# LarsDoorenbos/ccdm-stochastic-segmentation

Hardware: AMD Instinct MI355X
Metric: segmentation samples/sec, LIDC 128x128 T=250 (higher is better)
Workload: dtype f32 (conv products as split fp16 hi/lo x3 on MFMA, fp32 accumulate)

## Files before the change

### ccdm_stochastic_segmentation_amd/csrc/ccdm_conv.hip

```cpp
#include "ccdm_common.h"
#include "ccdm_conv_common.h"

#include <cmath>
#include <cstdlib>
#include <type_traits>
#include <vector>

namespace ccdm {


constexpr int min_waves(int mi, int ni, int prec, int ckt, int threads) {
    if (threads > 512) return 3;
    if (prec != CCDM_PREC_F32 && ckt >= 32) return 2;
    return mi * ni <= 2 ? 3 : (mi * ni <= 4 ? 2 : 1);
}

template <int PREC, int CKT, int KS, int STRIDE, int TH, int TW, int WAVES, int MI, int NI, int KSP = 1, bool UP2 = false, bool SKWT = false>
__global__ __launch_bounds__(WAVES * KSP * 64, min_waves(MI, NI, PREC, CKT, WAVES * KSP * 64)) void k_conv(const ConvK k) {
    constexpr int NT = WAVES * KSP * 64;
    static_assert(KSP == 1 || KSP == KS, "tap split is by kernel row");
    static_assert(!UP2 || (KS == 3 && STRIDE == 1 && KSP == 1 && (NI == 1 || NI == 4) && PREC != CCDM_PREC_F32), "sub-pixel form: 3x3, stride 1, F16X3, one phase or all four");
    constexpr int NTAP = UP2 ? 4 : KS * KS;
    constexpr int CK = CKT, PIXB = conv_pixb(PREC, CKT);
    constexpr int KST = CK / 16;
// ... 5 lines not shown
    constexpr int PXW = NT / QPP;
    static_assert(PXW % CW == 0, "a pass must cover whole core rows");
    constexpr int RPP = PXW / CW;
    constexpr int NCORE = (HHt + RPP - 1) / RPP;
    constexpr int ECOLS = HWt - CW > 0 ? HWt - CW : 1;
    constexpr int EDGE_ITEMS = HHt * (HWt - CW) * QPP;
    constexpr int NEDGE = (EDGE_ITEMS + NT - 1) / NT;
    constexpr bool ROW_UNIFORM = (CW * QPP) % 64 == 0;
    constexpr int NITEM = NCORE + NEDGE;
    static_assert(NITEM <= 32, "validity mask is 32 bits");
    constexpr bool SKW = SKWT && PREC != CCDM_PREC_F32 && KS == 3 && STRIDE == 1 && TW == 32 && NI == 1 && KSP == 1 && !UP2 && CKT == 16;
    constexpr int CKS = 32, PIXS = conv_pixb(CCDM_PREC_F16X3, CKS), QPS = CKS / 4;
    constexpr int NITEM_S = SKW ? TH * TW * QPS / NT : 0;
    constexpr int NITEM_R = NITEM_S > NITEM ? NITEM_S : NITEM;
    static_assert(!SKW || (TH * TW * QPS) % NT == 0, "a wide skip chunk tiles the block");
    constexpr int A_BYTES = (HP * PIXB + 15) / 16 * 16;
    constexpr int G = NI * FRAG_ITEMS;
    constexpr int NB4 = PREC == CCDM_PREC_F32 ? 0 : NTAP * KST * G;
    constexpr int NITEM_B = (NB4 + NT - 1) / NT;
    constexpr bool B_MULTI = NT % G == 0;
    static_assert(PREC == CCDM_PREC_F32 || B_MULTI || G % NT == 0, "B slabs must tile the block");
    constexpr int MB = B_MULTI ? NT / G : 1, DB = B_MULTI ? 1 : G / NT;

    const ccdm_conv_args& a = k.a;
    extern __shared__ __attribute__((aligned(16))) char smem[];
    const int C = a.C0 + a.C1;
    float2* ab = reinterpret_cast<float2*>(smem);
    char* halo_b = smem + (a.stats0 ? (size_t)C * 8 : 0);
    float* halo = reinterpret_cast<float*>(halo_b);
    f32x4* ldsB = reinterpret_cast<f32x4*>(halo_b + A_BYTES);
// ... 188 lines not shown
        const unsigned dst0 = (unsigned)(size_t)(skwc ? halo_b + TH * TW * PIXS : reinterpret_cast<char*>(ldsB));
        unsigned lane_ = lane;
        asm volatile("" : "+v"(lane_));
#pragma unroll
        for (int i = 0; i < MAXU; ++i) {
            const unsigned u = (unsigned)wave_all + (unsigned)(i * NWV);
            if (u < nunit) {
                const unsigned ts = u / UPS, part = u % UPS;
                const unsigned slab = skwc ? ts * wks : (ts / KST) * wtap + (ts % KST) * wks;
                const char* src = wq + (((size_t)slab + part * (FRAG_ITEMS / 2)) << 4) + (lane_ << 4);
                __builtin_amdgcn_global_load_lds(reinterpret_cast<const __attribute__((address_space(1))) void*>(reinterpret_cast<unsigned long long>(src)),
                                                 reinterpret_cast<__attribute__((address_space(3))) void*>(dst0 + u * (unsigned)(FRAG_BYTES / 2)), 16, 0, 0);
            }
        }
    };
    auto commit_body = [&](auto GN_, auto ACT_, int c0) {
        constexpr bool GN = decltype(GN_)::value, ACT = decltype(ACT_)::value;
        unsigned t_ = tid;
        asm volatile("" : "+v"(t_));
        const int tq = t_ % QPP, px = (t_ / QPP) % CW;
        float2 t0 = make_float2(1.f, 0.f), t1 = t0, t2 = t0, t3 = t0;
        if (GN) { const int c = c0 + 4 * tq; t0 = ab[c]; t1 = ab[c + 1]; t2 = ab[c + 2]; t3 = ab[c + 3]; }
        constexpr bool F16 = PREC != CCDM_PREC_F32;
        constexpr float PS = F16 ? ACT_PRESCALE : 1.0f;
        if (GN && !ACT && F16) { t0.x *= PS; t0.y *= PS; t1.x *= PS; t1.y *= PS; t2.x *= PS; t2.y *= PS; t3.x *= PS; t3.y *= PS; }
        auto act = [&](const float x) {
            if (!ACT) return (GN || !F16) ? x : x * PS;
            return x * __builtin_amdgcn_rcpf(1.0f / PS + __builtin_amdgcn_exp2f(fmaf(x, -1.4426950408889634f, F16 ? -4.0f : 0.0f)));
        };
        static_assert(ACT_PRESCALE == 16.0f, "the exp2 bias above is log2(ACT_PRESCALE)");
        auto put = [&](auto MASKED_, const f32x4 r, const bool ok, const int hp) {
            constexpr bool MASKED = decltype(MASKED_)::value;
// ... 46 lines not shown
        } else {
#pragma unroll
            for (int i = 0; i < NCORE; ++i)
                if ((i + 1) * RPP <= HHt || rip + i * RPP < HHt)
                    put(std::true_type{}, reg[i], xok[0] & (((rowmask[0] >> i) & 1u) != 0u), hp0 + i * RPP * HWt);
        }
#pragma unroll
        for (int j = 0; j < NEDGE; ++j) {
            const unsigned e = t_ + j * NT;
            if (e < (unsigned)EDGE_ITEMS) {
                const unsigned side = (e / QPP) % ECOLS, row = e / (ECOLS * QPP);
                const int hx = side < (unsigned)PAD ? (int)side : CW + (int)side;
                put(std::true_type{}, reg[NCORE + j], ((evalid[0] >> j) & 1u) != 0u, (int)row * HWt + hx);
            }
        }
        if (PREC != CCDM_PREC_F32 && !BDMA) {
#pragma unroll
            for (int i = 0; i < NITEM_B; ++i) {
                const int j = (int)t_ + i * NT;
                if ((i + 1) * NT <= NB4 || j < NB4) ldsB[j] = regB[i];
            }
        }
    };
    auto commit_skipw = [&]() {
        if constexpr (SKW) {
            unsigned t_ = tid;
            asm volatile("" : "+v"(t_));
            const int tq = t_ % QPS, px = t_ / QPS;
            typedef unsigned u32x2 __attribute__((ext_vector_type(2)));
#pragma unroll
            for (int i = 0; i < NITEM_S; ++i) {
// ... 2 lines not shown
                const float lim = ok ? __builtin_inff() : 0.f;
                const float v0 = __builtin_amdgcn_fmed3f(r[0] * ACT_PRESCALE, -lim, lim), v1 = __builtin_amdgcn_fmed3f(r[1] * ACT_PRESCALE, -lim, lim);
                const float v2 = __builtin_amdgcn_fmed3f(r[2] * ACT_PRESCALE, -lim, lim), v3 = __builtin_amdgcn_fmed3f(r[3] * ACT_PRESCALE, -lim, lim);
                u32x2 hi, lo;
                unsigned h0, l0, h1, l1;
                split2_f16(v0, v1, h0, l0);
                split2_f16(v2, v3, h1, l1);
                hi[0] = h0; hi[1] = h1; lo[0] = l0; lo[1] = l1;
                char* dd = halo_b + (i * TW + px) * PIXS + 8 * tq;
                *reinterpret_cast<u32x2*>(dd) = hi;
                *reinterpret_cast<u32x2*>(dd + 2 * CKS) = lo;
            }
            if (!BDMA) reinterpret_cast<f32x4*>(halo_b + TH * TW * PIXS)[t_] = regB[0];
        }
    };
    auto commit = [&](const int ch) {
        const bool sk = ch >= nchunk_main;
        if (SKW && skw && sk) { commit_skipw(); return; }
        const int c0 = (sk ? ch - nchunk_main : ch) * CK;
        const bool gn = has_gn && !sk, act = a.act == CCDM_ACT_SILU && !sk;
        if (gn && act) commit_body(std::true_type{}, std::true_type{}, c0);
        else if (gn) commit_body(std::true_type{}, std::false_type{}, c0);
        else if (act) commit_body(std::false_type{}, std::true_type{}, c0);
        else commit_body(std::false_type{}, std::false_type{}, c0);
    };

    f32x16 acc[MI][NI];
    const int adv_y = k.slices / k.tiles_x, adv_x = k.slices % k.tiles_x;
    auto advance = [&](int& ch, int& ty, int& tx) {
        if (++ch == nchunk) {
            ch = 0; tx += adv_x; ty += adv_y;
            if (tx >= k.tiles_x) { tx -= k.tiles_x; ++ty; }
        }
    };
    int chunk = 0, cur_ty = slice / k.tiles_x, cur_tx = slice % k.tiles_x;
    int pf_ch = 0, pf_ty = cur_ty, pf_tx = cur_tx;
    issue(pf_ch, pf_ty, pf_tx);
    advance(pf_ch, pf_ty, pf_tx);
    __builtin_amdgcn_sched_barrier(0);
#pragma unroll
    for (int ni = 0; ni < NI; ++ni) {
        const bool cv = tile_of(ni) * 32 + (lane & 31) < a.Cout;
        float add = a.bias ? raw_bias[ni] : 0.f;
        if (a.emb_off >= 0) add += raw_emb[ni];
        epi_add[ni] = (cv && krow == 0) ? add : 0.f;
        if (!cv) epi_wsc[ni] = 1.0f;
    }
    if (has_gn) gn_affine_block(a, n, emb_row, gpf, reinterpret_cast<f64x2*>(halo_b), ab, blockDim.x);
    auto iterate = [&]() {
        if (chunk == 0) {
#pragma unroll
            for (int mi = 0; mi < MI; ++mi)
#pragma unroll
                for (int ni = 0; ni < NI; ++ni)
#pragma unroll
                    for (int r = 0; r < 16; ++r) acc[mi][ni][r] = 0.0f;
        }
        issueB(chunk);
        __syncthreads();
        if constexpr (BDMA) {
#pragma unroll
            for (int i = 0; i < NITEM_R; ++i) asm volatile("" : "+v"(reg[i]));
            issueB_dma(chunk);
        }
        commit(chunk);
        __syncthreads();
        issue(pf_ch, pf_ty, pf_tx);
        advance(pf_ch, pf_ty, pf_tx);

        const bool skc = chunk >= nchunk_main;
        const int c0 = (skc ? chunk - nchunk_main : chunk) * CK;
        if (PREC == CCDM_PREC_F32) {
            const float* wc = reinterpret_cast<const float*>(skc ? a.skip_w : a.w) + ((size_t)(c0 >> 1) * k.ntiles + nt0) * 64 + lane;
            const size_t wtap = (size_t)(k.cin_pad >> 1) * k.ntiles * 64;
#pragma unroll
            for (int tap = 0; tap < KS * KS; ++tap) {
                if (skc && tap != (KS * KS) / 2) continue;
                const int toff = ((tap / KS) * HWt + (tap % KS)) * PIX_F32;
                const float* wt = wc + (skc ? 0 : tap * wtap);
#pragma unroll 4
                for (int kk = 0; kk < CK / 2; ++kk) {
                    float av[MI];
#pragma unroll
                    for (int mi = 0; mi < MI; ++mi) av[mi] = halo[base[mi] + toff + 2 * kk];
// ... 100 lines not shown
                            for (int mi = 0; mi < MI; ++mi) {
                                acc[mi][ni] = __builtin_amdgcn_mfma_f32_32x32x16_f16(al[0][mi], wh, acc[mi][ni], 0, 0, 0);
                                acc[mi][ni] = __builtin_amdgcn_mfma_f32_32x32x16_f16(ah[0][mi], wl, acc[mi][ni], 0, 0, 0);
                                acc[mi][ni] = __builtin_amdgcn_mfma_f32_32x32x16_f16(ah[0][mi], wh, acc[mi][ni], 0, 0, 0);
                            }
                        }
                    }
            } else if (UP2) {
                walk(std::integral_constant<int, 4>{}, [&](int t) { return ((t >> 1) * HWt + (t & 1)) * PIXB; }, [&](int t) { return t; });
            } else if (KSP > 1) {
                walk(std::integral_constant<int, KS>{}, [&](int u) { return (krow * HWt + u) * PIXB; }, [&](int u) { return krow * KS + u; });
            } else {
                walk(std::integral_constant<int, KS * KS>{}, [&](int tap) { return ((tap / KS) * HWt + (tap % KS)) * PIXB; }, [&](int tap) { return tap; });
            }
        }

        if (chunk == nchunk - 1) {
            const int oy0 = cur_ty * TH, ox0 = cur_tx * TW;
            int lane_ = lane;
            asm volatile("" : "+v"(lane_));
            if (fast_epi) {
                __syncthreads();
                const int cq = lane_ & 7, prow = lane_ >> 3;
#pragma unroll
                for (int ni = 0; ni < NI; ++ni) {
                    if (KSP > 1 && ni > 0) __syncthreads();
                    const int co4 = tile_of(ni) * 32 + 4 * cq;
                    const int dy = phase_of(ni) >> 1, dx = phase_of(ni) & 1;
                    const bool cv4 = co4 < a.Cout;
                    const int eH = UP2 ? Hc : aHout, eW = UP2 ? Wc : aWout;
                    const bool full = oy0 + TH <= eH && ox0 + TW <= eW && tile_of(ni) * 32 + 32 <= aCout;
                    constexpr int RS_FIRST = MI * 4 > 4 ? 4 : MI * 4;
                    f32x4 rs[MI * 4];
                    unsigned lane_off = ((unsigned)(UP2 ? 2 * prow : prow) * (unsigned)aCout + (unsigned)co4) << 2;
                    asm volatile("" : "+v"(lane_off));
                    auto row_of = [&](const int j) { return oy0 + wave * (MI * 32 / TW) + (j * 8) / TW; };
                    auto row_base = [&](const int j) {
                        if (UP2) return (unsigned)(((2 * row_of(j) + dy) * aWout + 2 * (ox0 + (j * 8) % TW) + dx) * aCout) << 2;
                        return (unsigned)((row_of(j) * aWout + ox0 + (j * 8) % TW) * aCout) << 2;
                    };
                    auto pix_of = [&](const int oy, const int ox) {
                        return UP2 ? (unsigned)((2 * oy + dy) * aWout + 2 * ox + dx) : (unsigned)(oy * aWout + ox);
                    };
                    double t1[4] = {0.0, 0.0, 0.0, 0.0}, t2[4] = {0.0, 0.0, 0.0, 0.0};
                    auto epi_ni = [&](auto FULL_, auto RESID_) {
                    constexpr bool FULL = decltype(FULL_)::value, RESID = decltype(RESID_)::value;
                    auto load_resid = [&](const int j0, const int j1) {
#pragma unroll
                        for (int j = j0; j < j1; ++j) {
                            if (KSP > 1 && j % KSP != krow) continue;
                            if (FULL) rs[j] = load16_uniform_base(reinterpret_cast<const char*>(residn) + row_base(j), lane_off);
                            else {
                                const int oy = min(row_of(j), eH - 1), ox = min(ox0 + (j * 8) % TW + prow, eW - 1);
                                const int cc = min(co4, aCout - 4);
                                rs[j] = *reinterpret_cast<const f32x4*>(reinterpret_cast<const char*>(residn) +
                                                                        ((pix_of(oy, ox) * (unsigned)aCout + (unsigned)cc) << 2));
                            }
                        }
                    };
                    if (RESID) load_resid(0, RS_FIRST);
                    constexpr bool EXACT3 = KS == 1 && RESID && PREC != CCDM_PREC_F32;
                    float addq[4] = {0.f, 0.f, 0.f, 0.f};
                    if (EXACT3) {
#pragma unroll
                        for (int e = 0; e < 4; ++e) addq[e] = __shfl(epi_add[ni], 4 * cq + e);
                    }
                    {
                        const float add = EXACT3 ? 0.f : epi_add[ni], wsc = epi_wsc[ni];
#pragma unroll
                        for (int mi = 0; mi < MI; ++mi)
#pragma unroll
                            for (int r = 0; r < 16; ++r) {
                                const int pl = mi * 32 + (r & 3) + 8 * (r >> 2) + 4 * (lane_ >> 5);
                                epi[pl * EPS + (lane_ & 31)] = PREC == CCDM_PREC_F32 ? acc[mi][ni][r] + add : fmaf(acc[mi][ni][r], wsc, add);
                            }
                    }
                    if (KSP > 1) __syncthreads();
                    const float* epi0 = reinterpret_cast<const float*>(halo_b) + wave * (MI * 32 * EPS);
                    {
#pragma unroll
                        for (int j = 0; j < MI * 4; ++j) {
                            if (j == RS_FIRST && RESID) load_resid(RS_FIRST, MI * 4);
                            if (KSP > 1 && j % KSP != krow) continue;
                            const int pl = j * 8 + prow;
                            f32x4 v = *reinterpret_cast<const f32x4*>(epi0 + pl * EPS + 4 * cq);
#pragma unroll
                            for (int g = 1; g < KSP; ++g)
                                v += *reinterpret_cast<const f32x4*>(epi0 + g * (WAVES * MI * 32 * EPS) + pl * EPS + 4 * cq);
                            if (EXACT3) {
#pragma unroll
                                for (int e = 0; e < 4; ++e) v[e] = (float)((double)v[e] + ((double)addq[e] + (double)rs[j][e]));
                            } else if (RESID) v += rs[j];
                            if (FULL) {
                                store16_uniform_base(reinterpret_cast<char*>(outn) + row_base(j), lane_off, v);
#pragma unroll
                                for (int e = 0; e < 4; ++e) { const double d = v[e]; t1[e] += d; t2[e] = fma(d, d, t2[e]); }
                            } else {
                                const int oy = row_of(j), ox = ox0 + (j * 8) % TW + prow;
                                if (cv4 && oy < eH && ox < eW) {
                                    *reinterpret_cast<f32x4*>(reinterpret_cast<char*>(outn) +
                                                              ((pix_of(oy, ox) * (unsigned)aCout + (unsigned)co4) << 2)) = v;
#pragma unroll
                                    for (int e = 0; e < 4; ++e) { const double d = v[e]; t1[e] += d; t2[e] = fma(d, d, t2[e]); }
                                }
                            }
                        }
                    }
                    };
                    if (a.resid) { if (full) epi_ni(std::true_type{}, std::true_type{}); else epi_ni(std::false_type{}, std::true_type{}); }
                    else { if (full) epi_ni(std::true_type{}, std::false_type{}); else epi_ni(std::false_type{}, std::false_type{}); }
                    {
                        const bool b2 = (lane_ >> 5) & 1, b1 = (lane_ >> 4) & 1, b0 = (lane_ >> 3) & 1;
                        double u[4], w[2];
#pragma unroll
                        for (int i = 0; i < 4; ++i) u[i] = (b2 ? t2[i] : t1[i]) + __shfl_xor(b2 ? t1[i] : t2[i], 32);
#pragma unroll
                        for (int i = 0; i < 2; ++i) w[i] = (b1 ? u[2 + i] : u[i]) + __shfl_xor(b1 ? u[i] : u[2 + i], 16);
                        st[ni] += (b0 ? w[1] : w[0]) + __shfl_xor(b0 ? w[0] : w[1], 8);
                    }
                }
            } else {
#pragma unroll
            for (int ni = 0; ni < NI; ++ni) {
                const int co = (nt0 + ni) * 32 + (lane_ & 31);
                const bool cv = co < a.Cout;
                const float add = epi_add[ni], wsc = epi_wsc[ni];
                double t1 = 0.0, t2 = 0.0;
#pragma unroll
                for (int mi = 0; mi < MI; ++mi) {
                    const int pb = (wave * MI + mi) * 32 + 4 * (lane_ >> 5);
#pragma unroll
                    for (int r = 0; r < 16; ++r) {
                        const int p = pb + (r & 3) + 8 * (r >> 2);
                        const int oy = oy0 + p / TW, ox = ox0 + p % TW;
                        if (cv && oy < a.Hout && ox < a.Wout) {
                            const size_t idx = ((size_t)(n * a.Hout + oy) * a.Wout + ox) * a.Cout + co;
                            float v;
                            if (KS == 1 && PREC != CCDM_PREC_F32 && a.resid) v = (float)((double)(acc[mi][ni][r] * wsc) + ((double)add + (double)a.resid[idx]));
                            else {
                                v = (PREC == CCDM_PREC_F32 ? acc[mi][ni][r] : acc[mi][ni][r] * wsc) + add;
                                if (a.resid) v += a.resid[idx];
                            }
                            a.out[idx] = v;
                            const double d = v;
                            t1 += d;
                            t2 = fma(d, d, t2);
                        }
                    }
                }
                const bool h = lane_ >> 5;
                st[ni] += (h ? t2 : t1) + __shfl_xor(h ? t1 : t2, 32);
            }
            }
        }
        advance(chunk, cur_ty, cur_tx);
    };
    for (int it = 0; it < n_iter; ++it) iterate();

    if (a.out_stats) {
        __syncthreads();
        double* red = reinterpret_cast<double*>(halo_b);
        const int ch = fast_epi ? 4 * (lane & 7) + ((lane >> 3) & 3) : lane & 31, comp = lane >> 5;
#pragma unroll
        for (int ni = 0; ni < NI; ++ni) red[((wave_all * NI + ni) * 32 + ch) * 2 + comp] = st[ni];
        __syncthreads();
        constexpr int NFOLD = UP2 && NI == 4 ? 4 : 1;
        for (int i = tid; i < NI / NFOLD * 32; i += NT) {
            const int ni = (i >> 5) * NFOLD, l = i & 31;
            double t1 = 0.0, t2 = 0.0;
            for (int f = 0; f < NFOLD; ++f) gn_fold_waves(red, ni + f, NI, WAVES * KSP, l, t1, t2);
            const int co = tile_of(ni) * 32 + l;
            if (co < a.Cout) {
// ... 183 lines not shown
        return 0;
    }
    if (conv1x1_eligible(a, p.slices)) {
        conv1x1_plan(a, p);
        return 0;
    }
    if (conv_takes_ks(a)) {
        CCDM_REQUIRE(conv_ks_describe(a, p), "conv_ks: geometry not built");
        return 0;
    }
    p.kernel = CCDM_CONV_KERNEL_GENERAL;
    const int HP = ((g.TH - 1) * a.stride + a.ksize) * ((g.TW - 1) * a.stride + a.ksize);
    const int ck = chunk_ck(a, g);
    p.chunk = ck;
    p.skip_wide = (a.skip0 && prec == CCDM_PREC_F16X3 && a.ksize == 3 && a.stride == 1 && !a.up && g.TW == 32 && NI == 1 && ck == 16 &&
                   a.SC0 % 32 == 0 && a.SC1 % 32 == 0 && !(a.prec >> 8)) ? 1 : 0;
    {
        const int SC = a.SC0 + a.SC1;
        const bool chan_ok = a.C0 % ck == 0 && a.C1 % ck == 0 && (!a.skip0 || (a.SC0 % ck == 0 && a.SC1 % ck == 0 && SC > 0));
        p.core_unmasked = ((up2 ? a.Win : Wc) % (g.TW * a.stride) == 0 && chan_ok) ? 1 : 0;
    }
    CCDM_REQUIRE(a.C1 == 0 || a.C0 % ck == 0, "conv: first source has %d channels; a concatenated input must split at a multiple of the %d-channel chunk", a.C0, ck);
    CCDM_REQUIRE(a.SC1 == 0 || a.SC0 % ck == 0, "conv: first skip source has %d channels; a concatenated input must split at a multiple of the %d-channel chunk", a.SC0, ck);
    CCDM_REQUIRE((p.cin_pad + p.cin_pad_skip) / ck <= 64, "conv: %d input (+%d skip) channels make more than 64 chunks of %d (chunk descriptors live in the 64 lanes of a register)",
                 p.cin_pad, p.cin_pad_skip, ck);
    size_t lds = (size_t)HP * conv_pixb(prec, ck);
    lds = (lds + 15) / 16 * 16;
    if (prec != CCDM_PREC_F32) lds += (size_t)(up2 ? 4 : a.ksize * a.ksize) * (ck / 16) * NI * FRAG_BYTES;
    p.tap_split = tap_split(a, g) ? 1 : 0;
    const int ksp = p.tap_split ? 3 : 1;
    const size_t red = (size_t)g.waves * ksp * NI * 32 * 16;
// ... 36 lines not shown
        if (rck) return rck;
        CCDM_CHECK_LAUNCH("conv_ks");
        return 0;
    }
    ConvK k;
    k.a = a;
    k.cin_pad = p.cin_pad;
    k.cin_pad_skip = p.cin_pad_skip;
    k.ntiles = p.ntiles;
    k.slices = p.slices;
    k.tiles_x = cdiv(a.up == 2 ? a.Win : a.Wout, p.g.TW);
    k.tiles_y = cdiv(a.up == 2 ? a.Hin : a.Hout, p.g.TH);
    k.skip_wide = p.skip_wide;
    k.wscale = wscale;
    k.core_unmasked = p.core_unmasked;
    const int prec = a.prec & 255;
    const dim3 grid(p.grid_x, p.grid_y);
    const int rc = prec == CCDM_PREC_F32 ? launch_prec<CCDM_PREC_F32>(k, p.g, p.ntiles_per_block, p.chunk, grid, (size_t)p.lds_bytes, s)
                   : prec == CCDM_PREC_F16 ? launch_prec<CCDM_PREC_F16>(k, p.g, p.ntiles_per_block, p.chunk, grid, (size_t)p.lds_bytes, s)
                                           : launch_prec<CCDM_PREC_F16X3>(k, p.g, p.ntiles_per_block, p.chunk, grid, (size_t)p.lds_bytes, s);
    if (rc) return rc;
    CCDM_CHECK_LAUNCH("conv");
    return 0;
}

}

extern "C" int ccdm_conv_slices(int Hout, int Wout, int stride, int ksize) {
    (void)ksize;
    return ccdm::conv_slices(Hout, Wout, stride);
// ... 115 lines not shown
```

### ccdm_stochastic_segmentation_amd/csrc/ccdm_conv1x1.hip

```cpp
#include "ccdm_common.h"
#include "ccdm_conv_common.h"

#include <cstdlib>

namespace ccdm {

__device__ __forceinline__ float epi_bias_resid(float acc, float wsc, float add, float rs, bool resid) {
    if (!resid) return fmaf(acc, wsc, add);
    return (float)fma((double)acc, (double)wsc, (double)add + (double)rs);
}

struct Conv1x1K {
    const float* in;
    const void* w;
    const float* wscale;
    const float* bias;
    const float* resid;
    float* out;
    double* out_stats;
    int C, Cout, HW, slices, ntiles, px_per_block;
    ccdm_conv_args a;
};

template <int KSB, int MAXT, bool GN>
// ... 202 lines not shown
        if (t + 1 >= ntb || nt + 1 >= nt_real) break;
        issueB(0, nt + 2);
        tile(1, nt + 1);
    }
}

static int conv1x1_px_per_block(const ccdm_conv_args& a, int slices) {
    const int HW = a.Hout * a.Wout;
    if (a.out_stats) return (HW % (slices * 32) == 0 && HW / slices <= 512) ? HW / slices : 0;
    for (int p = 128; p >= 32; p >>= 1)
        if (HW % p == 0) return p;
    return 0;
}

bool conv1x1_eligible(const ccdm_conv_args& a, int slices) {
    if (a.prec != CCDM_PREC_F16X3) return false;
    if (a.ksize != 1 || a.stride != 1 || a.up || a.act != CCDM_ACT_NONE || a.film || a.skip0 || a.emb_off >= 0 || a.in1) return false;
    const int HW = a.Hout * a.Wout;
    if (a.C0 % 16 || a.Cout % 32 || a.C0 > CCDM_MAX_CHANNELS) return false;
    const int ppb = conv1x1_px_per_block(a, slices);
    if (a.stats0 && ppb > 128) return false;
    return ppb > 0 && HW <= 16384;
}

void conv1x1_plan(const ccdm_conv_args& a, ConvPlan& p) {
    const int HW = a.Hout * a.Wout, ppb = conv1x1_px_per_block(a, p.slices);
    p.slices = HW / ppb;
    p.tile_h = 1; p.tile_w = ppb;
    p.chunk = 16;
    p.block = ppb / 32 * 64;
    p.lds_bytes = a.stats0 ? a.C0 * 8 + (a.C0 > p.block ? a.C0 : p.block) * 16 : 0;
// ... 38 lines not shown
```

### ccdm_stochastic_segmentation_amd/csrc/ccdm_conv_common.h

```cpp
#pragma once
#include "ccdm_common.h"
#include "ccdm_gn.h"

namespace ccdm {

static constexpr float ACT_PRESCALE = 16.0f;

constexpr int PIX_F32 = 33;
constexpr int conv_pixb(int prec, int ck) { return prec == CCDM_PREC_F32 ? PIX_F32 * 4 : ck * 4 + 16; }
constexpr int EPI_ROW = 36;
constexpr int FRAG_ITEMS = 128, FRAG_BYTES = FRAG_ITEMS * 16;

typedef const __attribute__((address_space(1))) char* gptr_t;
__device__ __forceinline__ f32x4 load16_uniform_base(const char* base, unsigned voff) {
    const unsigned long long v = reinterpret_cast<unsigned long long>(base);
    const unsigned lo = __builtin_amdgcn_readfirstlane((unsigned)v), hi = __builtin_amdgcn_readfirstlane((unsigned)(v >> 32));
    gptr_t g = reinterpret_cast<gptr_t>(((unsigned long long)hi << 32) | lo);
    return *reinterpret_cast<const __attribute__((address_space(1))) f32x4*>(g + voff);
}

__device__ __forceinline__ f32x4 load16_global(const char* p) {
    return *reinterpret_cast<const __attribute__((address_space(1))) f32x4*>(reinterpret_cast<unsigned long long>(p));
}

// ... 8 lines not shown
__device__ __forceinline__ void split2_f16(const float a, const float b, unsigned& hi, unsigned& lo) {
    float la, lb;
    asm("v_cvt_pk_f16_f32 %0, %1, %2" : "=v"(hi) : "v"(a), "v"(b));
    asm("v_fma_mix_f32 %0, %1, -1.0, %2 op_sel:[0,0,0] op_sel_hi:[1,0,0]" : "=v"(la) : "v"(hi), "v"(a));
    asm("v_fma_mix_f32 %0, %1, -1.0, %2 op_sel:[1,0,0] op_sel_hi:[1,0,0]" : "=v"(lb) : "v"(hi), "v"(b));
    asm("v_cvt_pk_f16_f32 %0, %1, %2" : "=v"(lo) : "v"(la), "v"(lb));
}

struct ConvK {
    ccdm_conv_args a;
    int cin_pad, ntiles, slices, tiles_x, tiles_y;
    int cin_pad_skip;
    int skip_wide;
    const float* wscale;
    int core_unmasked;
};

struct ConvPlan : ccdm_conv_plan_info {
    ConvGeo g;
    int cin_pad, cin_pad_skip;
    size_t wscale_off;
};
int conv_plan(const ccdm_conv_args& a, ConvPlan& p);

bool conv1x1_eligible(const ccdm_conv_args& a, int slices);
void conv1x1_plan(const ccdm_conv_args& a, ConvPlan& p);
int launch_conv1x1(const ccdm_conv_args& a, const ConvPlan& p, const float* wscale, hipStream_t s);

bool conv_ks_eligible(const ccdm_conv_args& a);
int conv_ks_slices(const ccdm_conv_args& a);
// ... 8 lines not shown
```

### ccdm_stochastic_segmentation_amd/csrc/ccdm_conv_ks.hip

```cpp
#include "ccdm_common.h"
#include "ccdm_conv_common.h"

namespace ccdm {

struct ConvKS {
    ccdm_conv_args a;
    const float* wscale;
    int ntiles;
    int tiles_x, tiles_y;
    int C, SC;
    int nks_m, nks_s;
    int pitch_m, pitch_s;
    int lgq_m, lgq_s;
    int nit_m, nit_s;
    int skip_off;
    int nstep;
    int red_off;
};

constexpr int KS_NT = 512, KS_NW = 8, KS_PART_BYTES = 8 * 2 * 4 * 64 * 16;
constexpr int ks_bq(int ni) { return ni == 1 ? 10 : (ni == 2 ? 6 : (ni == 3 ? 4 : 2)); }

template <int STRIDE, bool GNACT, int NITM, int NITS, int NI = 1>
__global__ __launch_bounds__(KS_NT, NI == 1 ? 2 : 1) void k_conv_ks(const ConvKS k) {
// ... 344 lines not shown

static int pow2_lg_quads(int nks) {
    const int q = 4 * nks;
    return q <= 16 ? 4 : (q <= 32 ? 5 : 6);
}

static int conv_ks_ni(const ccdm_conv_args& a) {
    if (a.Hout * a.Wout <= 128) return 1;
    const int nt = a.Cout / 32;
    for (int ni = 4; ni > 1; --ni)
        if (nt % ni == 0) return ni;
    return 1;
}

static bool conv_ks_plan(const ccdm_conv_args& a, ConvKS& k, size_t& lds, int& NI) {
    if (a.prec != CCDM_PREC_F16X3) return false;
    if (a.ksize != 3 || a.up || a.film || (a.stride != 1 && a.stride != 2)) return false;
    if ((a.stats0 != nullptr) != (a.act == CCDM_ACT_SILU)) return false;
    if (a.Hout % 8 || a.Wout % 8 || a.Hout * a.Wout > 256) return false;
    if (a.Cout % 32) return false;
    const int C = a.C0 + a.C1, SC = a.skip0 ? a.SC0 + a.SC1 : 0;
    if (C > 256 || SC > 256 || (a.stride == 2 && a.skip0)) return false;
    NI = conv_ks_ni(a);
    if (NI > 1 && ((a.stride == 1) != (a.stats0 != nullptr))) return false;
    k.a = a;
    k.C = C; k.SC = SC;
    k.nks_m = cdiv(C, 16); k.nks_s = cdiv(SC, 16);
    k.pitch_m = conv_pixb(CCDM_PREC_F16X3, 16 * k.nks_m); k.pitch_s = conv_pixb(CCDM_PREC_F16X3, 16 * k.nks_s);
    k.lgq_m = pow2_lg_quads(k.nks_m); k.lgq_s = SC ? pow2_lg_quads(k.nks_s) : 6;
    const int HWt = 7 * a.stride + 3, HP = HWt * HWt;
    k.nit_m = cdiv(cdiv(HP, 64 >> k.lgq_m), KS_NW);
// ... 76 lines not shown
```

### ccdm_stochastic_segmentation_amd/csrc/ccdm_upconv.hip

```cpp
#include "ccdm_common.h"
#include "ccdm_conv_common.h"

#include <algorithm>

namespace ccdm {

struct UpK {
    const float* in;
    const void* w;
    const float* wscale;
    const float* bias;
    float* out;
    double* out_stats;
    int N, Hin, Win, Cout, ntiles, slices, tiles_x, tiles_y, ctb;
};

constexpr int UP_TH = 8, UP_HH = UP_TH + 2;
constexpr int UP_EPI_BYTES = 4 * 32 * EPI_ROW * 4;
constexpr int UP_CTB_MAX = 2;
constexpr int UP_BD = 2;

template <int C, int TW> struct UpGeo {
    static constexpr int PIXB = conv_pixb(CCDM_PREC_F16X3, C), QPP = C / 4, KS16 = C / 16, NF = KS16 * 4;
    static constexpr int HW = TW + 2, HP = UP_HH * HW, MT = UP_TH * TW / 32;
// ... 173 lines not shown
                o[1] = red[((w * UP_CTB_MAX + c) * 32 + l) * 2 + 1];
            }
        } else {
            for (int i = tid; i < k.ctb * 32; i += 256) {
                const int c = i >> 5, l = i & 31;
                double a1 = 0.0, a2 = 0.0;
                gn_fold_waves(red, c, UP_CTB_MAX, 4, l, a1, a2);
                double* o = k.out_stats + (((size_t)n * k.slices + slice) * Cout + (ct0 + c) * 32 + l) * 2;
                o[0] = a1; o[1] = a2;
            }
        }
    }
}

bool upconv_eligible(const ccdm_conv_args& a) {
    if (a.prec != CCDM_PREC_F16X3 || a.up != 2) return false;
    if (a.C1 || a.in1 || a.stats0 || a.act != CCDM_ACT_NONE || a.film || a.emb_off >= 0 || a.resid || a.skip0 || a.fine_slices) return false;
    if (!(a.C0 == 32 || a.C0 == 64 || a.C0 == 96 || a.C0 == 128) || a.Cout % 32) return false;
    return a.Hin % UP_TH == 0 && (a.Win % 16 == 0 || a.Win == 8);
}

void upconv_plan(const ccdm_conv_args& a, ConvPlan& p) {
    p.kernel = CCDM_CONV_KERNEL_UPCONV;
    p.tile_h = UP_TH; p.tile_w = a.Win == 8 ? 8 : 16;
    p.chunk = a.C0;
    const int ctiles = a.Cout / 32;
    p.ntiles_per_block = (ctiles % 2 == 0 && (long)a.N * p.slices * (ctiles / 2) >= 512) ? 2 : 1;
    p.grid_x = a.N * p.slices; p.grid_y = ctiles / p.ntiles_per_block; p.block = 256;
    const int a_bytes = UP_HH * (p.tile_w + 2) * conv_pixb(CCDM_PREC_F16X3, a.C0);
    p.lds_bytes = p.ntiles_per_block == 1 ? std::max(a_bytes, UP_EPI_BYTES) : a_bytes + UP_EPI_BYTES;
}
// ... 39 lines not shown
```

### ccdm_stochastic_segmentation_amd/hip.py

```python
from __future__ import annotations

import ctypes as C
import os
import subprocess
from typing import Optional

_HERE = os.path.dirname(os.path.abspath(__file__))
ROOT = os.path.dirname(_HERE)
LIB_PATH = os.environ.get("CCDM_LIB") or os.path.join(_HERE, "libccdm_hip.so")
CSRC = os.path.join(_HERE, "csrc")
SOURCES = ["ccdm_conv.hip", "ccdm_conv_ks.hip", "ccdm_upconv.hip", "ccdm_stem.hip", "ccdm_head.hip", "ccdm_conv1x1.hip", "ccdm_misc.hip", "ccdm_attention.hip", "ccdm_attn_block.hip", "ccdm_sampler.hip", "ccdm_known.hip", "ccdm_guided.hip", "ccdm_metrics.hip", "ccdm_range.hip", "ccdm_resample.hip", "ccdm_engine.hip", "ccdm_vote.hip", "ccdm_segeval.hip", "ccdm_segexport.hip", "ccdm_csscore.hip", "ccdm_segcalib.hip", "ccdm_segboundary.hip", "ccdm_contourf.hip", "ccdm_uncscore.hip", "ccdm_lidcscore.hip", "ccdm_surfdist.hip", "ccdm_lesions.hip", "ccdm_lesionmatch.hip", "ccdm_findings.hip", "ccdm_modes.hip", "ccdm_consensus.hip", "ccdm_bound.hip"]
HIPCC_FLAGS = ["--offload-arch=gfx950", "-O3", "-std=c++17", "-ffp-contract=off", "-mllvm", "-amdgpu-mfma-vgpr-form=1", "-fPIC", "-shared"]

ACT_NONE, ACT_SILU = 0, 1
RESAMPLE_AVGPOOL2, RESAMPLE_NEAREST_UP2 = 0, 1
ATTENTION_FORCE_VALU = 256
ATTENTION_VALU_WIDTHS = (4, 8, 12, 16, 24, 32, 48, 64)
DIAG_GENERAL_KERNEL = 2048 << 8
PREC_F32, PREC_F16X3 = 0, 1
PREC_F16 = 2
STEP_SAMPLE, STEP_LAST_CONFIDENCE, STEP_LAST_MAJORITY, STEP_LAST_KEEP, STEP_SOFTMAX_ONLY = 0, 1, 2, 3, 4
SLOT_IDLE = -1
SLOT_GUIDE_EVIDENCE, SLOT_GUIDE_KNOWN = 1, 2
BOUND_IDLE = -1
STATS_MAX_SLICES = 64
F16X3_LIMIT = 4094.0
STATS_FOLD_SLICES = 16
ABI_VERSION = 11
MAX_CLASSES = 255
CSSCORE_MAX_LABELS = 64
POST_DIAG_MANY = 256


# ... 435 lines not shown
```

### include/ccdm_hip.h

```cpp
#ifndef CCDM_HIP_H
#define CCDM_HIP_H

#include <stddef.h>
#include <stdint.h>

#ifdef __cplusplus
extern "C" {
#endif

#define CCDM_ABI_VERSION 11
#define CCDM_MAX_CHANNELS 1024
#define CCDM_STATS_MAX_SLICES 64
#define CCDM_STATS_FOLD_SLICES 16

int ccdm_version(void);
const char* ccdm_last_error_string(void);

int ccdm_gn_stats(const float* x , int N, int HW, int C, int slices,
                  double* stats , void* stream);

enum { CCDM_ACT_NONE = 0, CCDM_ACT_SILU = 1 };
enum { CCDM_PREC_F32 = 0,
       CCDM_PREC_F16X3 = 1,
       CCDM_PREC_F16 = 2 };

#define CCDM_DIAG_GENERAL_KERNEL (2048 << 8)

typedef struct ccdm_conv_args {
    const float* in0; const float* in1; int32_t C0; int32_t C1;
    const double* stats0; const double* stats1; int32_t slices0; int32_t slices1;
    const float* gamma; const float* beta;
    float eps; int32_t act;
    int32_t film; int32_t film_off;
    int32_t N, Hin, Win, Hout, Wout;
    int32_t ksize;
    int32_t stride;
    int32_t up;
    const void* w; const float* bias; int32_t Cout; int32_t prec;
    const float* emb_table; int32_t emb_stride; int32_t emb_off;
    const int32_t* emb_row_of_sample;
    const int32_t* step_ptr;
// ... 355 lines not shown
```

Before: 95.00.

## Process two output tiles per weight chunk to reuse staged weights in conv

For F16X3 3x3 stride-1 convs with TW=32, MI=2, NI=1, the tile loop now walks tile pairs. Each channel chunk's weight slab is staged into LDS once and used for both tiles, which keep separate accumulators. This removes the repeated weight writeback for the second tile, at the cost of doubling accumulator registers, which can reduce occupancy. A diagnostic flag restores the single-tile walk, and the other eligibility checks mask that flag out.

```diff
diff --git a/ccdm_stochastic_segmentation_amd/csrc/ccdm_conv.hip b/ccdm_stochastic_segmentation_amd/csrc/ccdm_conv.hip
--- a/ccdm_stochastic_segmentation_amd/csrc/ccdm_conv.hip
+++ b/ccdm_stochastic_segmentation_amd/csrc/ccdm_conv.hip
@@ -43,6 +43,7 @@
     constexpr int NITEM_S = SKW ? TH * TW * QPS / NT : 0;
     constexpr int NITEM_R = NITEM_S > NITEM ? NITEM_S : NITEM;
     static_assert(!SKW || (TH * TW * QPS) % NT == 0, "a wide skip chunk tiles the block");
+    constexpr bool PAIR = PREC == CCDM_PREC_F16X3 && CKT == 16 && KS == 3 && STRIDE == 1 && TW == 32 && MI == 2 && NI == 1 && KSP == 1 && !UP2 && !SKWT;
     constexpr int A_BYTES = (HP * PIXB + 15) / 16 * 16;
     constexpr int G = NI * FRAG_ITEMS;
     constexpr int NB4 = PREC == CCDM_PREC_F32 ? 0 : NTAP * KST * G;
@@ -261,8 +262,8 @@
             }
         }
     };
-    auto commit_body = [&](auto GN_, auto ACT_, int c0) {
-        constexpr bool GN = decltype(GN_)::value, ACT = decltype(ACT_)::value;
+    auto commit_body = [&](auto GN_, auto ACT_, auto WB_, int c0) {
+        constexpr bool GN = decltype(GN_)::value, ACT = decltype(ACT_)::value, WB = decltype(WB_)::value;
         unsigned t_ = tid;
         asm volatile("" : "+v"(t_));
         const int tq = t_ % QPP, px = (t_ / QPP) % CW;
@@ -339,7 +340,7 @@
                 put(std::true_type{}, reg[NCORE + j], ((evalid[0] >> j) & 1u) != 0u, (int)row * HWt + hx);
             }
         }
-        if (PREC != CCDM_PREC_F32 && !BDMA) {
+        if (PREC != CCDM_PREC_F32 && !BDMA && WB) {
 #pragma unroll
             for (int i = 0; i < NITEM_B; ++i) {
                 const int j = (int)t_ + i * NT;
@@ -372,18 +373,18 @@
             if (!BDMA) reinterpret_cast<f32x4*>(halo_b + TH * TW * PIXS)[t_] = regB[0];
         }
     };
-    auto commit = [&](const int ch) {
+    auto commit = [&](const int ch, auto WB_) {
         const bool sk = ch >= nchunk_main;
         if (SKW && skw && sk) { commit_skipw(); return; }
         const int c0 = (sk ? ch - nchunk_main : ch) * CK;
         const bool gn = has_gn && !sk, act = a.act == CCDM_ACT_SILU && !sk;
-        if (gn && act) commit_body(std::true_type{}, std::true_type{}, c0);
-        else if (gn) commit_body(std::true_type{}, std::false_type{}, c0);
-        else if (act) commit_body(std::false_type{}, std::true_type{}, c0);
-        else commit_body(std::false_type{}, std::false_type{}, c0);
+        if (gn && act) commit_body(std::true_type{}, std::true_type{}, WB_, c0);
+        else if (gn) commit_body(std::true_type{}, std::false_type{}, WB_, c0);
+        else if (act) commit_body(std::false_type{}, std::true_type{}, WB_, c0);
+        else commit_body(std::false_type{}, std::false_type{}, WB_, c0);
     };
 
-    f32x16 acc[MI][NI];
+    f32x16 accs[PAIR ? 2 : 1][MI][NI];
     const int adv_y = k.slices / k.tiles_x, adv_x = k.slices % k.tiles_x;
     auto advance = [&](int& ch, int& ty, int& tx) {
         if (++ch == nchunk) {
@@ -391,7 +392,7 @@
             if (tx >= k.tiles_x) { tx -= k.tiles_x; ++ty; }
         }
     };
-    int chunk = 0, cur_ty = slice / k.tiles_x, cur_tx = slice % k.tiles_x;
+    int cur_ch = 0, cur_ty = slice / k.tiles_x, cur_tx = slice % k.tiles_x;
     int pf_ch = 0, pf_ty = cur_ty, pf_tx = cur_tx;
     issue(pf_ch, pf_ty, pf_tx);
     advance(pf_ch, pf_ty, pf_tx);
@@ -405,27 +406,28 @@
         if (!cv) epi_wsc[ni] = 1.0f;
     }
     if (has_gn) gn_affine_block(a, n, emb_row, gpf, reinterpret_cast<f64x2*>(halo_b), ab, blockDim.x);
-    auto iterate = [&]() {
-        if (chunk == 0) {
-#pragma unroll
-            for (int mi = 0; mi < MI; ++mi)
-#pragma unroll
-                for (int ni = 0; ni < NI; ++ni)
-#pragma unroll
-                    for (int r = 0; r < 16; ++r) acc[mi][ni][r] = 0.0f;
-        }
-        issueB(chunk);
+    auto clear = [&](auto& acc) {
+#pragma unroll
+        for (int mi = 0; mi < MI; ++mi)
+#pragma unroll
+            for (int ni = 0; ni < NI; ++ni)
+#pragma unroll
+                for (int r = 0; r < 16; ++r) acc[mi][ni][r] = 0.0f;
+    };
+    auto stage = [&](auto SECOND_, const int chunk, auto&& prefetch) {
+        constexpr bool SECOND = decltype(SECOND_)::value;
+        if (!SECOND) issueB(chunk);
         __syncthreads();
         if constexpr (BDMA) {
 #pragma unroll
             for (int i = 0; i < NITEM_R; ++i) asm volatile("" : "+v"(reg[i]));
             issueB_dma(chunk);
         }
-        commit(chunk);
+        commit(chunk, std::integral_constant<bool, !SECOND>{});
         __syncthreads();
-        issue(pf_ch, pf_ty, pf_tx);
-        advance(pf_ch, pf_ty, pf_tx);
-
+        prefetch();
+    };
+    auto matrix = [&](auto& acc, const int chunk) {
         const bool skc = chunk >= nchunk_main;
         const int c0 = (skc ? chunk - nchunk_main : chunk) * CK;
         if (PREC == CCDM_PREC_F32) {
@@ -556,148 +558,184 @@
                 walk(std::integral_constant<int, KS * KS>{}, [&](int tap) { return ((tap / KS) * HWt + (tap % KS)) * PIXB; }, [&](int tap) { return tap; });
             }
         }
-
-        if (chunk == nchunk - 1) {
-            const int oy0 = cur_ty * TH, ox0 = cur_tx * TW;
-            int lane_ = lane;
-            asm volatile("" : "+v"(lane_));
-            if (fast_epi) {
-                __syncthreads();
-                const int cq = lane_ & 7, prow = lane_ >> 3;
-#pragma unroll
-                for (int ni = 0; ni < NI; ++ni) {
-                    if (KSP > 1 && ni > 0) __syncthreads();
-                    const int co4 = tile_of(ni) * 32 + 4 * cq;
-                    const int dy = phase_of(ni) >> 1, dx = phase_of(ni) & 1;
-                    const bool cv4 = co4 < a.Cout;
-                    const int eH = UP2 ? Hc : aHout, eW = UP2 ? Wc : aWout;
-                    const bool full = oy0 + TH <= eH && ox0 + TW <= eW && tile_of(ni) * 32 + 32 <= aCout;
-                    constexpr int RS_FIRST = MI * 4 > 4 ? 4 : MI * 4;
-                    f32x4 rs[MI * 4];
-                    unsigned lane_off = ((unsigned)(UP2 ? 2 * prow : prow) * (unsigned)aCout + (unsigned)co4) << 2;
-                    asm volatile("" : "+v"(lane_off));
-                    auto row_of = [&](const int j) { return oy0 + wave * (MI * 32 / TW) + (j * 8) / TW; };
-                    auto row_base = [&](const int j) {
-                        if (UP2) return (unsigned)(((2 * row_of(j) + dy) * aWout + 2 * (ox0 + (j * 8) % TW) + dx) * aCout) << 2;
-                        return (unsigned)((row_of(j) * aWout + ox0 + (j * 8) % TW) * aCout) << 2;
-                    };
-                    auto pix_of = [&](const int oy, const int ox) {
-                        return UP2 ? (unsigned)((2 * oy + dy) * aWout + 2 * ox + dx) : (unsigned)(oy * aWout + ox);
-                    };
-                    double t1[4] = {0.0, 0.0, 0.0, 0.0}, t2[4] = {0.0, 0.0, 0.0, 0.0};
-                    auto epi_ni = [&](auto FULL_, auto RESID_) {
-                    constexpr bool FULL = decltype(FULL_)::value, RESID = decltype(RESID_)::value;
-                    auto load_resid = [&](const int j0, const int j1) {
-#pragma unroll
-                        for (int j = j0; j < j1; ++j) {
-                            if (KSP > 1 && j % KSP != krow) continue;
-                            if (FULL) rs[j] = load16_uniform_base(reinterpret_cast<const char*>(residn) + row_base(j), lane_off);
-                            else {
-                                const int oy = min(row_of(j), eH - 1), ox = min(ox0 + (j * 8) % TW + prow, eW - 1);
-                                const int cc = min(co4, aCout - 4);
-                                rs[j] = *reinterpret_cast<const f32x4*>(reinterpret_cast<const char*>(residn) +
-                                                                        ((pix_of(oy, ox) * (unsigned)aCout + (unsigned)cc) << 2));
-                            }
+    };
+    auto epilogue = [&](auto& acc, const int ty, const int tx) {
+        const int oy0 = ty * TH, ox0 = tx * TW;
+        int lane_ = lane;
+        asm volatile("" : "+v"(lane_));
+        if (fast_epi) {
+            __syncthreads();
+            const int cq = lane_ & 7, prow = lane_ >> 3;
+#pragma unroll
+            for (int ni = 0; ni < NI; ++ni) {
+                if (KSP > 1 && ni > 0) __syncthreads();
+                const int co4 = tile_of(ni) * 32 + 4 * cq;
+                const int dy = phase_of(ni) >> 1, dx = phase_of(ni) & 1;
+                const bool cv4 = co4 < a.Cout;
+                const int eH = UP2 ? Hc : aHout, eW = UP2 ? Wc : aWout;
+                const bool full = oy0 + TH <= eH && ox0 + TW <= eW && tile_of(ni) * 32 + 32 <= aCout;
+                constexpr int RS_FIRST = MI * 4 > 4 ? 4 : MI * 4;
+                f32x4 rs[MI * 4];
+                unsigned lane_off = ((unsigned)(UP2 ? 2 * prow : prow) * (unsigned)aCout + (unsigned)co4) << 2;
+                asm volatile("" : "+v"(lane_off));
+                auto row_of = [&](const int j) { return oy0 + wave * (MI * 32 / TW) + (j * 8) / TW; };
+                auto row_base = [&](const int j) {
+                    if (UP2) return (unsigned)(((2 * row_of(j) + dy) * aWout + 2 * (ox0 + (j * 8) % TW) + dx) * aCout) << 2;
+                    return (unsigned)((row_of(j) * aWout + ox0 + (j * 8) % TW) * aCout) << 2;
+                };
+                auto pix_of = [&](const int oy, const int ox) {
+                    return UP2 ? (unsigned)((2 * oy + dy) * aWout + 2 * ox + dx) : (unsigned)(oy * aWout + ox);
+                };
+                double t1[4] = {0.0, 0.0, 0.0, 0.0}, t2[4] = {0.0, 0.0, 0.0, 0.0};
+                auto epi_ni = [&](auto FULL_, auto RESID_) {
+                constexpr bool FULL = decltype(FULL_)::value, RESID = decltype(RESID_)::value;
+                auto load_resid = [&](const int j0, const int j1) {
+#pragma unroll
+                    for (int j = j0; j < j1; ++j) {
+                        if (KSP > 1 && j % KSP != krow) continue;
+                        if (FULL) rs[j] = load16_uniform_base(reinterpret_cast<const char*>(residn) + row_base(j), lane_off);
+                        else {
+                            const int oy = min(row_of(j), eH - 1), ox = min(ox0 + (j * 8) % TW + prow, eW - 1);
+                            const int cc = min(co4, aCout - 4);
+                            rs[j] = *reinterpret_cast<const f32x4*>(reinterpret_cast<const char*>(residn) +
+                                                                    ((pix_of(oy, ox) * (unsigned)aCout + (unsigned)cc) << 2));
                         }
-                    };
-                    if (RESID) load_resid(0, RS_FIRST);
-                    constexpr bool EXACT3 = KS == 1 && RESID && PREC != CCDM_PREC_F32;
-                    float addq[4] = {0.f, 0.f, 0.f, 0.f};
-                    if (EXACT3) {
-#pragma unroll
-                        for (int e = 0; e < 4; ++e) addq[e] = __shfl(epi_add[ni], 4 * cq + e);
                     }
-                    {
-                        const float add = EXACT3 ? 0.f : epi_add[ni], wsc = epi_wsc[ni];
-#pragma unroll
-                        for (int mi = 0; mi < MI; ++mi)
-#pragma unroll
-                            for (int r = 0; r < 16; ++r) {
-                                const int pl = mi * 32 + (r & 3) + 8 * (r >> 2) + 4 * (lane_ >> 5);
-                                epi[pl * EPS + (lane_ & 31)] = PREC == CCDM_PREC_F32 ? acc[mi][ni][r] + add : fmaf(acc[mi][ni][r], wsc, add);
-                            }
-                    }
-                    if (KSP > 1) __syncthreads();
-                    const float* epi0 = reinterpret_cast<const float*>(halo_b) + wave * (MI * 32 * EPS);
-                    {
-#pragma unroll
-                        for (int j = 0; j < MI * 4; ++j) {
-                            if (j == RS_FIRST && RESID) load_resid(RS_FIRST, MI * 4);
-                            if (KSP > 1 && j % KSP != krow) continue;
-                            const int pl = j * 8 + prow;
-                            f32x4 v = *reinterpret_cast<const f32x4*>(epi0 + pl * EPS + 4 * cq);
-#pragma unroll
-                            for (int g = 1; g < KSP; ++g)
-                                v += *reinterpret_cast<const f32x4*>(epi0 + g * (WAVES * MI * 32 * EPS) + pl * EPS + 4 * cq);
-                            if (EXACT3) {
-#pragma unroll
-                                for (int e = 0; e < 4; ++e) v[e] = (float)((double)v[e] + ((double)addq[e] + (double)rs[j][e]));
-                            } else if (RESID) v += rs[j];
-                            if (FULL) {
-                                store16_uniform_base(reinterpret_cast<char*>(outn) + row_base(j), lane_off, v);
+                };
+                if (RESID) load_resid(0, RS_FIRST);
+                constexpr bool EXACT3 = KS == 1 && RESID && PREC != CCDM_PREC_F32;
+                float addq[4] = {0.f, 0.f, 0.f, 0.f};
+                if (EXACT3) {
+#pragma unroll
+                    for (int e = 0; e < 4; ++e) addq[e] = __shfl(epi_add[ni], 4 * cq + e);
+                }
+                {
+                    const float add = EXACT3 ? 0.f : epi_add[ni], wsc = epi_wsc[ni];
+#pragma unroll
+                    for (int mi = 0; mi < MI; ++mi)
+#pragma unroll
+                        for (int r = 0; r < 16; ++r) {
+                            const int pl = mi * 32 + (r & 3) + 8 * (r >> 2) + 4 * (lane_ >> 5);
+                            epi[pl * EPS + (lane_ & 31)] = PREC == CCDM_PREC_F32 ? acc[mi][ni][r] + add : fmaf(acc[mi][ni][r], wsc, add);
+                        }
+                }
+                if (KSP > 1) __syncthreads();
+                const float* epi0 = reinterpret_cast<const float*>(halo_b) + wave * (MI * 32 * EPS);
+                {
+#pragma unroll
+                    for (int j = 0; j < MI * 4; ++j) {
+                        if (j == RS_FIRST && RESID) load_resid(RS_FIRST, MI * 4);
+                        if (KSP > 1 && j % KSP != krow) continue;
+                        const int pl = j * 8 + prow;
+                        f32x4 v = *reinterpret_cast<const f32x4*>(epi0 + pl * EPS + 4 * cq);
+#pragma unroll
+                        for (int g = 1; g < KSP; ++g)
+                            v += *reinterpret_cast<const f32x4*>(epi0 + g * (WAVES * MI * 32 * EPS) + pl * EPS + 4 * cq);
+                        if (EXACT3) {
+#pragma unroll
+                            for (int e = 0; e < 4; ++e) v[e] = (float)((double)v[e] + ((double)addq[e] + (double)rs[j][e]));
+                        } else if (RESID) v += rs[j];
+                        if (FULL) {
+                            store16_uniform_base(reinterpret_cast<char*>(outn) + row_base(j), lane_off, v);
+#pragma unroll
+                            for (int e = 0; e < 4; ++e) { const double d = v[e]; t1[e] += d; t2[e] = fma(d, d, t2[e]); }
+                        } else {
+                            const int oy = row_of(j), ox = ox0 + (j * 8) % TW + prow;
+                            if (cv4 && oy < eH && ox < eW) {
+                                *reinterpret_cast<f32x4*>(reinterpret_cast<char*>(outn) +
+                                                          ((pix_of(oy, ox) * (unsigned)aCout + (unsigned)co4) << 2)) = v;
 #pragma unroll
                                 for (int e = 0; e < 4; ++e) { const double d = v[e]; t1[e] += d; t2[e] = fma(d, d, t2[e]); }
-                            } else {
-                                const int oy = row_of(j), ox = ox0 + (j * 8) % TW + prow;
-                                if (cv4 && oy < eH && ox < eW) {
-                                    *reinterpret_cast<f32x4*>(reinterpret_cast<char*>(outn) +
-                                                              ((pix_of(oy, ox) * (unsigned)aCout + (unsigned)co4) << 2)) = v;
-#pragma unroll
-                                    for (int e = 0; e < 4; ++e) { const double d = v[e]; t1[e] += d; t2[e] = fma(d, d, t2[e]); }
-                                }
                             }
                         }
                     }
-                    };
-                    if (a.resid) { if (full) epi_ni(std::true_type{}, std::true_type{}); else epi_ni(std::false_type{}, std::true_type{}); }
-                    else { if (full) epi_ni(std::true_type{}, std::false_type{}); else epi_ni(std::false_type{}, std::false_type{}); }
-                    {
-                        const bool b2 = (lane_ >> 5) & 1, b1 = (lane_ >> 4) & 1, b0 = (lane_ >> 3) & 1;
-                        double u[4], w[2];
-#pragma unroll
-                        for (int i = 0; i < 4; ++i) u[i] = (b2 ? t2[i] : t1[i]) + __shfl_xor(b2 ? t1[i] : t2[i], 32);
-#pragma unroll
-                        for (int i = 0; i < 2; ++i) w[i] = (b1 ? u[2 + i] : u[i]) + __shfl_xor(b1 ? u[i] : u[2 + i], 16);
-                        st[ni] += (b0 ? w[1] : w[0]) + __shfl_xor(b0 ? w[0] : w[1], 8);
+                }
+                };
+                if (a.resid) { if (full) epi_ni(std::true_type{}, std::true_type{}); else epi_ni(std::false_type{}, std::true_type{}); }
+                else { if (full) epi_ni(std::true_type{}, std::false_type{}); else epi_ni(std::false_type{}, std::false_type{}); }
+                {
+                    const bool b2 = (lane_ >> 5) & 1, b1 = (lane_ >> 4) & 1, b0 = (lane_ >> 3) & 1;
+                    double u[4], w[2];
+#pragma unroll
+                    for (int i = 0; i < 4; ++i) u[i] = (b2 ? t2[i] : t1[i]) + __shfl_xor(b2 ? t1[i] : t2[i], 32);
+#pragma unroll
+                    for (int i = 0; i < 2; ++i) w[i] = (b1 ? u[2 + i] : u[i]) + __shfl_xor(b1 ? u[i] : u[2 + i], 16);
+                    st[ni] += (b0 ? w[1] : w[0]) + __shfl_xor(b0 ? w[0] : w[1], 8);
+                }
+            }
+        } else {
+#pragma unroll
+        for (int ni = 0; ni < NI; ++ni) {
+            const int co = (nt0 + ni) * 32 + (lane_ & 31);
+            const bool cv = co < a.Cout;
+            const float add = epi_add[ni], wsc = epi_wsc[ni];
+            double t1 = 0.0, t2 = 0.0;
+#pragma unroll
+            for (int mi = 0; mi < MI; ++mi) {
+                const int pb = (wave * MI + mi) * 32 + 4 * (lane_ >> 5);
+#pragma unroll
+                for (int r = 0; r < 16; ++r) {
+                    const int p = pb + (r & 3) + 8 * (r >> 2);
+                    const int oy = oy0 + p / TW, ox = ox0 + p % TW;
+                    if (cv && oy < a.Hout && ox < a.Wout) {
+                        const size_t idx = ((size_t)(n * a.Hout + oy) * a.Wout + ox) * a.Cout + co;
+                        float v;
+                        if (KS == 1 && PREC != CCDM_PREC_F32 && a.resid) v = (float)((double)(acc[mi][ni][r] * wsc) + ((double)add + (double)a.resid[idx]));
+                        else {
+                            v = (PREC == CCDM_PREC_F32 ? acc[mi][ni][r] : acc[mi][ni][r] * wsc) + add;
+                            if (a.resid) v += a.resid[idx];
+                        }
+                        a.out[idx] = v;
+                        const double d = v;
+                        t1 += d;
+                        t2 = fma(d, d, t2);
                     }
                 }
-            } else {
-#pragma unroll
-            for (int ni = 0; ni < NI; ++ni) {
-                const int co = (nt0 + ni) * 32 + (lane_ & 31);
-                const bool cv = co < a.Cout;
-                const float add = epi_add[ni], wsc = epi_wsc[ni];
-                double t1 = 0.0, t2 = 0.0;
-#pragma unroll
-                for (int mi = 0; mi < MI; ++mi) {
-                    const int pb = (wave * MI + mi) * 32 + 4 * (lane_ >> 5);
-#pragma unroll
-                    for (int r = 0; r < 16; ++r) {
-                        const int p = pb + (r & 3) + 8 * (r >> 2);
-                        const int oy = oy0 + p / TW, ox = ox0 + p % TW;
-                        if (cv && oy < a.Hout && ox < a.Wout) {
-                            const size_t idx = ((size_t)(n * a.Hout + oy) * a.Wout + ox) * a.Cout + co;
-                            float v;
-                            if (KS == 1 && PREC != CCDM_PREC_F32 && a.resid) v = (float)((double)(acc[mi][ni][r] * wsc) + ((double)add + (double)a.resid[idx]));
-                            else {
-                                v = (PREC == CCDM_PREC_F32 ? acc[mi][ni][r] : acc[mi][ni][r] * wsc) + add;
-                                if (a.resid) v += a.resid[idx];
-                            }
-                            a.out[idx] = v;
-                            const double d = v;
-                            t1 += d;
-                            t2 = fma(d, d, t2);
-                        }
-                    }
-                }
-                const bool h = lane_ >> 5;
-                st[ni] += (h ? t2 : t1) + __shfl_xor(h ? t1 : t2, 32);
-            }
-            }
-        }
-        advance(chunk, cur_ty, cur_tx);
+            }
+            const bool h = lane_ >> 5;
+            st[ni] += (h ? t2 : t1) + __shfl_xor(h ? t1 : t2, 32);
+        }
+        }
     };
-    for (int it = 0; it < n_iter; ++it) iterate();
+    if constexpr (!PAIR) {
+        for (int it = 0; it < n_iter; ++it) {
+            if (cur_ch == 0) clear(accs[0]);
+            stage(std::false_type{}, cur_ch, [&]() { issue(pf_ch, pf_ty, pf_tx); advance(pf_ch, pf_ty, pf_tx); });
+            matrix(accs[0], cur_ch);
+            if (cur_ch == nchunk - 1) epilogue(accs[0], cur_ty, cur_tx);
+            advance(cur_ch, cur_ty, cur_tx);
+        }
+    } else {
+        auto next_tile = [&](int& ty, int& tx) {
+            tx += adv_x; ty += adv_y;
+            if (tx >= k.tiles_x) { tx -= k.tiles_x; ++ty; }
+        };
+        const bool pairs = k.tile_pairs != 0;
+        int ta_ty = cur_ty, ta_tx = cur_tx;
+        for (int t = 0; t < my_tiles;) {
+            const bool two = pairs && t + 1 < my_tiles;
+            int tb_ty = ta_ty, tb_tx = ta_tx;
+            next_tile(tb_ty, tb_tx);
+            int nx_ty = tb_ty, nx_tx = tb_tx;
+            if (two) next_tile(nx_ty, nx_tx);
+            for (int ch = 0; ch < nchunk; ++ch) {
+                const bool last = ch == nchunk - 1;
+                const int up_ch = last ? 0 : ch + 1, up_ty = last ? nx_ty : ta_ty, up_tx = last ? nx_tx : ta_tx;
+                if (ch == 0) clear(accs[0]);
+                stage(std::false_type{}, ch, [&]() { issue(two ? ch : up_ch, two ? tb_ty : up_ty, two ? tb_tx : up_tx); });
+                matrix(accs[0], ch);
+                if (two) {
+                    if (ch == 0) clear(accs[1]);
+                    stage(std::true_type{}, ch, [&]() { issue(up_ch, up_ty, up_tx); });
+                    matrix(accs[1], ch);
+                }
+            }
+            epilogue(accs[0], ta_ty, ta_tx);
+            if (two) epilogue(accs[1], tb_ty, tb_tx);
+            ta_ty = nx_ty; ta_tx = nx_tx;
+            t += two ? 2 : 1;
+        }
+    }
 
     if (a.out_stats) {
         __syncthreads();
@@ -911,7 +949,7 @@
     const int ck = chunk_ck(a, g);
     p.chunk = ck;
     p.skip_wide = (a.skip0 && prec == CCDM_PREC_F16X3 && a.ksize == 3 && a.stride == 1 && !a.up && g.TW == 32 && NI == 1 && ck == 16 &&
-                   a.SC0 % 32 == 0 && a.SC1 % 32 == 0 && !(a.prec >> 8)) ? 1 : 0;
+                   a.SC0 % 32 == 0 && a.SC1 % 32 == 0 && !((a.prec & ~CCDM_DIAG_SINGLE_TILE_WALK) >> 8)) ? 1 : 0;
     {
         const int SC = a.SC0 + a.SC1;
         const bool chan_ok = a.C0 % ck == 0 && a.C1 % ck == 0 && (!a.skip0 || (a.SC0 % ck == 0 && a.SC1 % ck == 0 && SC > 0));
@@ -978,6 +1016,7 @@
     k.skip_wide = p.skip_wide;
     k.wscale = wscale;
     k.core_unmasked = p.core_unmasked;
+    k.tile_pairs = (a.prec & CCDM_DIAG_SINGLE_TILE_WALK) ? 0 : 1;
     const int prec = a.prec & 255;
     const dim3 grid(p.grid_x, p.grid_y);
     const int rc = prec == CCDM_PREC_F32 ? launch_prec<CCDM_PREC_F32>(k, p.g, p.ntiles_per_block, p.chunk, grid, (size_t)p.lds_bytes, s)
diff --git a/ccdm_stochastic_segmentation_amd/csrc/ccdm_conv1x1.hip b/ccdm_stochastic_segmentation_amd/csrc/ccdm_conv1x1.hip
--- a/ccdm_stochastic_segmentation_amd/csrc/ccdm_conv1x1.hip
+++ b/ccdm_stochastic_segmentation_amd/csrc/ccdm_conv1x1.hip
@@ -240,7 +240,7 @@
 }
 
 bool conv1x1_eligible(const ccdm_conv_args& a, int slices) {
-    if (a.prec != CCDM_PREC_F16X3) return false;
+    if ((a.prec & ~CCDM_DIAG_SINGLE_TILE_WALK) != CCDM_PREC_F16X3) return false;
     if (a.ksize != 1 || a.stride != 1 || a.up || a.act != CCDM_ACT_NONE || a.film || a.skip0 || a.emb_off >= 0 || a.in1) return false;
     const int HW = a.Hout * a.Wout;
     if (a.C0 % 16 || a.Cout % 32 || a.C0 > CCDM_MAX_CHANNELS) return false;
diff --git a/ccdm_stochastic_segmentation_amd/csrc/ccdm_conv_common.h b/ccdm_stochastic_segmentation_amd/csrc/ccdm_conv_common.h
--- a/ccdm_stochastic_segmentation_amd/csrc/ccdm_conv_common.h
+++ b/ccdm_stochastic_segmentation_amd/csrc/ccdm_conv_common.h
@@ -46,6 +46,7 @@
     int skip_wide;
     const float* wscale;
     int core_unmasked;
+    int tile_pairs;
 };
 
 struct ConvPlan : ccdm_conv_plan_info {
diff --git a/ccdm_stochastic_segmentation_amd/csrc/ccdm_conv_ks.hip b/ccdm_stochastic_segmentation_amd/csrc/ccdm_conv_ks.hip
--- a/ccdm_stochastic_segmentation_amd/csrc/ccdm_conv_ks.hip
+++ b/ccdm_stochastic_segmentation_amd/csrc/ccdm_conv_ks.hip
@@ -382,7 +382,7 @@
 }
 
 static bool conv_ks_plan(const ccdm_conv_args& a, ConvKS& k, size_t& lds, int& NI) {
-    if (a.prec != CCDM_PREC_F16X3) return false;
+    if ((a.prec & ~CCDM_DIAG_SINGLE_TILE_WALK) != CCDM_PREC_F16X3) return false;
     if (a.ksize != 3 || a.up || a.film || (a.stride != 1 && a.stride != 2)) return false;
     if ((a.stats0 != nullptr) != (a.act == CCDM_ACT_SILU)) return false;
     if (a.Hout % 8 || a.Wout % 8 || a.Hout * a.Wout > 256) return false;
diff --git a/ccdm_stochastic_segmentation_amd/csrc/ccdm_upconv.hip b/ccdm_stochastic_segmentation_amd/csrc/ccdm_upconv.hip
--- a/ccdm_stochastic_segmentation_amd/csrc/ccdm_upconv.hip
+++ b/ccdm_stochastic_segmentation_amd/csrc/ccdm_upconv.hip
@@ -211,7 +211,7 @@
 }
 
 bool upconv_eligible(const ccdm_conv_args& a) {
-    if (a.prec != CCDM_PREC_F16X3 || a.up != 2) return false;
+    if ((a.prec & ~CCDM_DIAG_SINGLE_TILE_WALK) != CCDM_PREC_F16X3 || a.up != 2) return false;
     if (a.C1 || a.in1 || a.stats0 || a.act != CCDM_ACT_NONE || a.film || a.emb_off >= 0 || a.resid || a.skip0 || a.fine_slices) return false;
     if (!(a.C0 == 32 || a.C0 == 64 || a.C0 == 96 || a.C0 == 128) || a.Cout % 32) return false;
     return a.Hin % UP_TH == 0 && (a.Win % 16 == 0 || a.Win == 8);
diff --git a/ccdm_stochastic_segmentation_amd/hip.py b/ccdm_stochastic_segmentation_amd/hip.py
--- a/ccdm_stochastic_segmentation_amd/hip.py
+++ b/ccdm_stochastic_segmentation_amd/hip.py
@@ -17,6 +17,7 @@
 ATTENTION_FORCE_VALU = 256
 ATTENTION_VALU_WIDTHS = (4, 8, 12, 16, 24, 32, 48, 64)
 DIAG_GENERAL_KERNEL = 2048 << 8
+DIAG_SINGLE_TILE_WALK = 4096 << 8
 PREC_F32, PREC_F16X3 = 0, 1
 PREC_F16 = 2
 STEP_SAMPLE, STEP_LAST_CONFIDENCE, STEP_LAST_MAJORITY, STEP_LAST_KEEP, STEP_SOFTMAX_ONLY = 0, 1, 2, 3, 4
diff --git a/include/ccdm_hip.h b/include/ccdm_hip.h
--- a/include/ccdm_hip.h
+++ b/include/ccdm_hip.h
@@ -25,6 +25,7 @@
        CCDM_PREC_F16 = 2 };
 
 #define CCDM_DIAG_GENERAL_KERNEL (2048 << 8)
+#define CCDM_DIAG_SINGLE_TILE_WALK (4096 << 8)
 
 typedef struct ccdm_conv_args {
     const float* in0; const float* in1; int32_t C0; int32_t C1;
```

Result: slower. 91.43 (-3.8%).
